# AIS-Bonn/stillleben

Measured on AMD Instinct MI355X. Metric: scenes/sec (settle + 640x480 6-ch GT render), 20-obj YCB-like, higher is better.
Workload: dtype f32; 1 GPU; C2: 20 of 21 procedural YCB-like objects (8k verts/16k tris, 1024^2 texture each) per scene; per step and GPU 32768 scenes are staged (random stack), settled (100 frames x 4 substeps), framed (camera, light, shadow matrix) and rendered at 640x480 (rgb, coord+depth, class, instance, normals; shadows on, SSAO on) -- all four stages inside the timed region; render_chunk=512, objects=20, settle_streams=1, render_streams=2, pair_contact_budget=0, parallelism=1 GPU

## Files before the change

### stillleben_amd/csrc/slhip_render.hip

```cpp
#include <vector>
#include <type_traits>
#include "slhip_common.h"
#include "slhip_cubemap.h"

#ifndef SLHIP_RENDER_WAVES
#define SLHIP_RENDER_WAVES 0
#endif
#ifndef SLHIP_SHADE_WAVES
#define SLHIP_SHADE_WAVES 0
#endif
#ifndef SLHIP_SSAO_WAVES
#define SLHIP_SSAO_WAVES 0
#endif
#if SLHIP_RENDER_WAVES > 0
#define SLHIP_LIGHT_KERNEL __attribute__((amdgpu_waves_per_eu(1, SLHIP_RENDER_WAVES)))
#else
#define SLHIP_LIGHT_KERNEL
#endif
#if SLHIP_SSAO_WAVES > 0
#define SLHIP_SSAO_KERNEL __attribute__((amdgpu_waves_per_eu(1, SLHIP_SSAO_WAVES)))
#else
#define SLHIP_SSAO_KERNEL
#endif
#if SLHIP_SHADE_WAVES > 0
// ... 996 lines not shown
                                                      const float4* __restrict__ clipbuf, unsigned n_clip_verts, int nl)
{
    const unsigned count = min(queue[0], capacity);
    const QItem* items = reinterpret_cast<const QItem*>(queue + 4);
    const unsigned lane = threadIdx.x & 63;
    const unsigned wave = (blockIdx.x * blockDim.x + threadIdx.x) >> 6;
    const unsigned n_waves = (gridDim.x * blockDim.x) >> 6;
    const unsigned per = (count + n_waves - 1) / n_waves;
    const unsigned i0 = wave * per, i1 = min(i0 + per, count);
    unsigned p_draw = 0xFFFFFFFFu, p_tri = 0u, p_scene = 0u;
    bool ok = false;
    Setup t;
    for (unsigned i = i0; i < i1; ++i) {
        const QItem it = items[i];
        if (it.draw == 0xFFFFFFFFu) continue;
        const unsigned scene = it.scene_aux & 0xFFFFFFu;
        const int light = (int)(it.scene_aux >> 24);
        if (it.draw != p_draw || it.tri_sub != p_tri || it.scene_aux != p_scene) {
            p_draw = it.draw; p_tri = it.tri_sub; p_scene = it.scene_aux;
            ok = false;
            const slhip_draw* dr = draws + it.draw;
            const unsigned* ip = pool.d_idx + dr->idx_base + 3 * (size_t)it.tri_sub;
            const float4* plane = clipbuf + (size_t)(1 + light) * n_clip_verts + dr->clip_base;
            const uint4* sp = reinterpret_cast<const uint4*>(plane);
            if (!setup_from_screen(sp[ip[0]], sp[ip[1]], sp[ip[2]], S, S, t)) continue;
            ok = true;
        }
        if (!ok) continue;
        const int px = (int)((it.tile & 0xFFFFu) << 3) + (int)(lane & 7);
        const int py = (int)((it.tile >> 16) << 3) + (int)(lane >> 3);
        if (px < t.xmin || px > t.xmax || py < t.ymin || py > t.ymax) continue;
        float l[3];
        if (!coverage(t, px, py, l)) continue;
        ShadowTarget tgt;
        tgt.win = nullptr; tgt.wx0 = 0; tgt.wy0 = 0;
        tgt.sm = shadow + ((size_t)scene * nl + light) * S * S;
        tgt.W = S;
        tgt.emit(t, px, py, l);
    }
}

__device__ __forceinline__ float frcp(float x) { return __builtin_amdgcn_rcpf(x); }
__device__ __forceinline__ void normalize3_fast(float* v)
{
    const float r = __builtin_amdgcn_rsqf(fmaf(v[2], v[2], fmaf(v[1], v[1], v[0] * v[0])));
    v[0] *= r; v[1] *= r; v[2] *= r;
}

__device__ __forceinline__ float distribution_ggx(const float* N, const float* Hv, float roughness)
{
    const float a = roughness * roughness;
    const float a2 = a * a;
    const float NdotH = fmaxf(dot3(N, Hv), 0.0f);
    const float NdotH2 = NdotH * NdotH;
    float denom = (NdotH2 * (a2 - 1.0f) + 1.0f);
    denom = kPi * denom * denom;
    return a2 * frcp(denom);
}

__device__ __forceinline__ float geometry_schlick_ggx(float NdotV, float roughness)
{
    const float r = roughness + 1.0f;
    const float k = (r * r) * 0.125f;
    return NdotV * frcp(NdotV * (1.0f - k) + k);
}

__device__ __forceinline__ float shadow_tap(const float* __restrict__ sm, int S, float u, float v, float ref)
{
    const float x = fmaf(u, (float)S, -0.5f), y = fmaf(v, (float)S, -0.5f);
    const float fx = floorf(x), fy = floorf(y);
    const float ax = x - fx, ay = y - fy;
    int x0 = (int)fx, y0 = (int)fy, x1 = x0 + 1, y1 = y0 + 1;
    x0 = min(max(x0, 0), S - 1); x1 = min(max(x1, 0), S - 1);
    y0 = min(max(y0, 0), S - 1); y1 = min(max(y1, 0), S - 1);
    const float r = clampf(ref, 0.0f, 1.0f);
    const float c00 = r <= sm[(size_t)y0 * S + x0] ? 1.0f : 0.0f;
    const float c10 = r <= sm[(size_t)y0 * S + x1] ? 1.0f : 0.0f;
    const float c01 = r <= sm[(size_t)y1 * S + x0] ? 1.0f : 0.0f;
    const float c11 = r <= sm[(size_t)y1 * S + x1] ? 1.0f : 0.0f;
    const float top = fmaf(ax, c10 - c00, c00), bot = fmaf(ax, c11 - c01, c01);
    return fmaf(ay, bot - top, top);
}

__device__ __forceinline__ float shadow_pcf16(const float* __restrict__ sm, int S, float px, float py, float ref,
                                              const unsigned* __restrict__ tile_bits)
{
    const float scale = 1.0f / (float)S;
    int ix[4], iy[4];
    float ax[4], ay[4];
    bool regular = true;
#pragma unroll
    for (int k = 0; k < 4; ++k) {
        const float o = (-1.5f + (float)k) * scale;
        const float x = fmaf(px + o, (float)S, -0.5f), y = fmaf(py + o, (float)S, -0.5f);
        const float fx = floorf(x), fy = floorf(y);
        ax[k] = x - fx; ay[k] = y - fy;
        ix[k] = (int)fx; iy[k] = (int)fy;
        if (k > 0 && (ix[k] != ix[0] + k || iy[k] != iy[0] + k)) regular = false;
    }
    float acc = 0.0f;
    if (regular) {
        const float r = clampf(ref, 0.0f, 1.0f);
        unsigned off_y[5];
        int cx[5];
#pragma unroll
        for (int k = 0; k < 5; ++k) {
            cx[k] = min(max(ix[0] + k, 0), S - 1);
            off_y[k] = (unsigned)min(max(iy[0] + k, 0), S - 1) * (unsigned)S;
        }
        if (tile_bits) {
            const int tn = shadow_tiles_x(S);
            const int ta = cx[0] / kShadowTile, tb = cx[4] / kShadowTile;
            const int ra = (int)(off_y[0] / (unsigned)S) / kShadowTile, rb = (int)(off_y[4] / (unsigned)S) / kShadowTile;
            const int t00 = ra * tn + ta, t01 = ra * tn + tb, t10 = rb * tn + ta, t11 = rb * tn + tb;
            const unsigned touched = ((tile_bits[t00 >> 5] >> (t00 & 31)) | (tile_bits[t01 >> 5] >> (t01 & 31)) |
                                      (tile_bits[t10 >> 5] >> (t10 & 31)) | (tile_bits[t11 >> 5] >> (t11 & 31))) & 1u;
            if (__ballot(touched == 0u) == __ballot(true)) return 1.0f;
        }
        bool lit[5][5];
        unsigned long long all_lit = ~0ull, any_lit = 0ull;
#pragma unroll
        for (int j = 0; j < 5; ++j)
#pragma unroll
            for (int i = 0; i < 5; ++i) {
                lit[j][i] = r <= sm[off_y[j] + (unsigned)cx[i]];
                const unsigned long long m = __ballot(lit[j][i]);
                all_lit &= m; any_lit |= m;
            }
        const unsigned long long here = __ballot(true);
        if (all_lit == here) return 1.0f;
        if (any_lit == 0ull) return 0.0f;
        float c[5][5];
#pragma unroll
        for (int j = 0; j < 5; ++j)
#pragma unroll
            for (int i = 0; i < 5; ++i) c[j][i] = lit[j][i] ? 1.0f : 0.0f;
#pragma unroll
        for (int yy = 0; yy < 4; ++yy)
#pragma unroll
            for (int xx = 0; xx < 4; ++xx) {
                const float top = fmaf(ax[xx], c[yy][xx + 1] - c[yy][xx], c[yy][xx]);
                const float bot = fmaf(ax[xx], c[yy + 1][xx + 1] - c[yy + 1][xx], c[yy + 1][xx]);
                acc += fmaf(ay[yy], bot - top, top);
            }
    } else {
        for (int yy = 0; yy < 4; ++yy)
            for (int xx = 0; xx < 4; ++xx) {
                const float ox = (-1.5f + (float)xx) * scale, oy = (-1.5f + (float)yy) * scale;
                acc += shadow_tap(sm, S, px + ox, py + oy, ref);
            }
    }
    return acc / 16.0f;
}

__device__ __forceinline__ float pow22(float x) { return __builtin_amdgcn_exp2f(2.2f * __builtin_amdgcn_logf(x)); }

__device__ __forceinline__ void shade_fragment(const slhip_scene* __restrict__ sc, const slhip_draw* __restrict__ dr,
                                               const float* base, const float* world, const float* nrm_in,
                                               bool front_facing, const float* __restrict__ shadow, int S, int shadow_lights,
                                               const unsigned* __restrict__ shadow_tiles, const slhip_light_map* __restrict__ lm, float roughness_in, float metallic_in,
                                               float occlusion, const float* emissive, float* color, float* normal_out)
{
    float normal[3] = {nrm_in[0], nrm_in[1], nrm_in[2]};
    if (!front_facing) { normal[0] = -normal[0]; normal[1] = -normal[1]; normal[2] = -normal[2]; }
    float V[3] = {sc->cam_position[0] - world[0], sc->cam_position[1] - world[1],
                  sc->cam_position[2] - world[2]};
    normalize3(V);
    const float NoV = clampf(dot3(normal, V), 1e-5f, 1.0f);
    const float roughness = fmaxf(roughness_in, 0.045f);
    const float metallic = metallic_in;

    color[0] = color[1] = color[2] = 0.0f;
    color[3] = base[3];

    float F0[3], kS[3];
    const float om = 1.0f - NoV, om2 = om * om;
    const float p5 = om2 * om2 * om;
#pragma unroll
    for (int c = 0; c < 3; ++c) {
        F0[c] = 0.04f * (1.0f - metallic) + base[c] * metallic;
        const float Fr = fmaxf(1.0f - roughness, F0[c]) - F0[c];
        kS[c] = F0[c] + Fr * p5;
    }
    const float base_pi[3] = {base[0] * (1.0f / kPi), base[1] * (1.0f / kPi), base[2] * (1.0f / kPi)};
    for (int i = 0; i < SLHIP_NUM_LIGHTS; ++i) {
        if (!light_active(sc, i)) continue;
        const float* lc = sc->light_color[i];
        const float* ld = sc->light_dir[i];
        float inverse_shadow = 1.0f;
        if (shadow && i < shadow_lights) {
            const float w4[4] = {world[0], world[1], world[2], 1.0f};
            float pc[4];
            mv4(sc->shadow_mat[i], w4, pc);
            const float rpw = 1.0f / pc[3];
            const float px = fmaf(pc[0] * rpw, 0.5f, 0.5f);
            const float py = fmaf(pc[1] * rpw, 0.5f, 0.5f);
            const float pz = fmaf(pc[2] * rpw, 0.5f, 0.5f);
            const float* sm = shadow + (size_t)i * S * S;
            inverse_shadow = shadow_pcf16(sm, S, px, py, (pz - 0.00003f), shadow_tiles ? shadow_tiles + (size_t)i * shadow_tile_words(S) : nullptr);
        }
        float L[3] = {-ld[0], -ld[1], -ld[2]};
        normalize3_fast(L);
        float Hv[3] = {V[0] + L[0], V[1] + L[1], V[2] + L[2]};
        normalize3_fast(Hv);
        const float NDF = distribution_ggx(normal, Hv, roughness);
        const float NdotVg = fmaxf(dot3(normal, V), 0.0f);
        const float NdotL = fmaxf(dot3(normal, L), 0.0f);
        const float G = geometry_schlick_ggx(NdotL, roughness) * geometry_schlick_ggx(NdotVg, roughness);
        const float denominator = fmaxf(4.0f * NoV * NdotL, 0.001f);
        const float rden = frcp(denominator);
#pragma unroll
        for (int c = 0; c < 3; ++c) {
            const float specular = (NDF * G * kS[c]) * rden;
            const float kD = (1.0f - kS[c]) * (1.0f - metallic);
            color[c] += inverse_shadow * (kD * base_pi[c] + specular) * lc[c] * NdotL;
        }
    }
#pragma unroll
    for (int c = 0; c < 3; ++c) color[c] += sc->ambient[c] * base[c];
    if (lm) {
        const float d2 = 2.0f * dot3(normal, V);
        const slcube::f3 refl = slcube::F3(d2 * normal[0] - V[0], d2 * normal[1] - V[1], d2 * normal[2] - V[2]);
        float fab[2];
        {
            const int n = (int)lm->lut_size;
            const float x = NoV * (float)n - 0.5f, y = roughness * (float)n - 0.5f;
            const float fx = floorf(x), fy = floorf(y);
            const float a = x - fx, b = y - fy;
            const int x0 = min(max((int)fx, 0), n - 1), x1 = min(max((int)fx + 1, 0), n - 1);
            const int y0 = min(max((int)fy, 0), n - 1), y1 = min(max((int)fy + 1, 0), n - 1);
            const float2* t = reinterpret_cast<const float2*>(lm->d_brdf_lut);
            const float2 c00 = t[y0 * n + x0], c10 = t[y0 * n + x1], c01 = t[y1 * n + x0], c11 = t[y1 * n + x1];
            const float tx = fmaf(a, c10.x - c00.x, c00.x), bx = fmaf(a, c11.x - c01.x, c01.x);
            const float ty = fmaf(a, c10.y - c00.y, c00.y), by = fmaf(a, c11.y - c01.y, c01.y);
            fab[0] = fmaf(b, bx - tx, tx); fab[1] = fmaf(b, by - ty, ty);
        }
        const float4 rad4 = slcube::sample_lod(lm->d_prefilter, lm->pre_size, lm->pre_levels, refl, roughness * 4.0f);
        const float4 irr4 = slcube::sample_lod(lm->d_irradiance, lm->irr_size, 1u, slcube::F3(normal[0], normal[1], normal[2]), 0.0f);
        const float rad[3] = {rad4.x, rad4.y, rad4.z}, irr[3] = {irr4.x, irr4.y, irr4.z};
        const float Ems = 1.0f - (fab[0] + fab[1]);
#pragma unroll
        for (int c = 0; c < 3; ++c) {
            const float c_diff = base[c] * (1.0f - 0.04f) * (1.0f - metallic);
            const float FssEss = kS[c] * fab[0] + fab[1];
            const float F_avg = F0[c] + (1.0f - F0[c]) / 21.0f;
            const float FmsEms = Ems * FssEss * F_avg / (1.0f - F_avg * Ems);
            const float k_D = c_diff * (1.0f - FssEss - FmsEms);
            color[c] += (FssEss * rad[c] + (FmsEms + k_D) * irr[c]) * occlusion;
        }
    }
#pragma unroll
    for (int c = 0; c < 3; ++c) color[c] += emissive[c];
    float nc[3];
#pragma unroll
    for (int r = 0; r < 3; ++r) {
        float a = fmaf(sc->world_to_cam[4 * r + 0], normal[0], 0.0f);
        a = fmaf(sc->world_to_cam[4 * r + 1], normal[1], a);
        a = fmaf(sc->world_to_cam[4 * r + 2], normal[2], a);
        nc[r] = a;
    }
    normalize3(nc);
    normal_out[0] = nc[0]; normal_out[1] = nc[1]; normal_out[2] = nc[2];
    normal_out[3] = dot3(normal, V);
}

__device__ __forceinline__ uchar4 tone_map_px(const float* c, float manual_exposure, float lum)
{
    const float X = 0.4124564f * c[0] + 0.3575761f * c[1] + 0.1804375f * c[2];
    float Y = 0.2126729f * c[0] + 0.7151522f * c[1] + 0.0721750f * c[2];
    const float Z = 0.0193339f * c[0] + 0.1191920f * c[1] + 0.9503041f * c[2];
    const float inv = frcp(X + Y + Z);
    const float xx = X * inv, yy = Y * inv;
    if (manual_exposure >= 0.0f) Y *= manual_exposure;
    else Y /= (9.6f * lum + 0.0001f);
    const float ryy = frcp(yy);
    const float x2 = Y * xx * ryy;
    const float y2 = Y;
    const float z2 = Y * (1.0f - xx - yy) * ryy;
    float o[3];
    o[0] = 3.2404542f * x2 + -1.5371385f * y2 + -0.4985314f * z2;
    o[1] = -0.9692660f * x2 + 1.8760108f * y2 + 0.0415560f * z2;
    o[2] = 0.0556434f * x2 + -0.2040259f * y2 + 1.0572252f * z2;
    unsigned char r[4];
#pragma unroll
    for (int k = 0; k < 3; ++k) {
        const float x = o[k];
        float v = (x * (2.51f * x + 0.03f)) * frcp(x * (2.43f * x + 0.59f) + 0.14f);
        v = fminf(fmaxf(v, 0.0f), 1.0f);
        if (!(v == v)) v = 0.0f;
        r[k] = (unsigned char)floorf(v * 255.0f + 0.5f);
    }
    const float a = fminf(fmaxf(c[3], 0.0f), 1.0f);
    r[3] = (unsigned char)floorf(a * 255.0f + 0.5f);
    return make_uchar4(r[0], r[1], r[2], r[3]);
}

__device__ __forceinline__ bool scene_block(unsigned blocks_per_scene, unsigned n_scenes, unsigned& scene, unsigned& blk)
{
    const unsigned x = blockIdx.x & 7u, j = blockIdx.x >> 3;
    scene = x + 8u * (j / blocks_per_scene);
    blk = j % blocks_per_scene;
    return scene < n_scenes;
}

struct PixelBary {
    float b[3], bx[3], by[3];
    bool front;
};
__device__ __forceinline__ bool resolve_pixel(const Setup& t, const float (&q0)[3], const float (&q1)[3], const float (&q2)[3],
                                              int px, int py, bool textured, PixelBary& r)
{
    float l[3];
    if (px < t.xmin || px > t.xmax || py < t.ymin || py > t.ymax) return false;
    if (!coverage(t, px, py, l)) return false;
    const float pw0 = l[0] * t.invw[0], pw1 = l[1] * t.invw[1], pw2 = l[2] * t.invw[2];
    const float sw = (pw0 + pw1) + pw2;
    const float bs[3] = {pw0 * (1.0f / sw), pw1 * (1.0f / sw), pw2 * (1.0f / sw)};
#pragma unroll
    for (int k = 0; k < 3; ++k) r.b[k] = fmaf(bs[2], q2[k], fmaf(bs[1], q1[k], bs[0] * q0[k]));
    r.front = t.flipped;
    if (textured) {
        bary_at(t, q0, q1, q2, px + 1, py, r.bx);
        bary_at(t, q0, q1, q2, px, py + 1, r.by);
    }
    return true;
}

struct ShadeParams {
    int W, H;
    unsigned n_scenes;
    unsigned flags;
    int S;
    int shadow_lights;
    int inline_tonemap;
    int want_lum;
    int tiled;
};

__global__ __launch_bounds__(256) SLHIP_SHADE_KERNEL void k_shade(slhip_mesh_pool pool, const slhip_scene* __restrict__ scenes,
                                               const slhip_draw* __restrict__ draws, ShadeParams prm,
                                               const unsigned long long* __restrict__ vis,
                                               slhip_render_out out, float* __restrict__ hdr,
                                               const float* __restrict__ shadow, float* __restrict__ lum_part,
                                               const float4* __restrict__ clipbuf, float* __restrict__ zplane,
                                               const float4* __restrict__ vattr, float2* __restrict__ ssao_tiles,
                                               const unsigned* __restrict__ shadow_tiles)
{
    const int W = prm.W, H = prm.H;
    const size_t P = (size_t)W * H;
    const unsigned blocks_per_scene = (unsigned)((P + 255) / 256);
    unsigned scene, blk;
    if (!scene_block(blocks_per_scene, prm.n_scenes, scene, blk)) return;
    unsigned pix;
    bool active;
    if (prm.tiled) {
        const unsigned per_row = (unsigned)W >> 5, l = threadIdx.x & 63u;
        const unsigned tx = (blk % per_row) * 32u + (threadIdx.x >> 6) * 8u + (l & 7u), ty = (blk / per_row) * 8u + (l >> 3);
        pix = ty * (unsigned)W + tx;
        active = true;
    } else {
        pix = blk * 256 + threadIdx.x;
        active = pix < P;
    }
    const slhip_scene* sc = scenes + scene;
    const size_t gp = (size_t)scene * P + pix;
    __shared__ unsigned s_prim_base[64];
    const unsigned n_scene_draws = sc->draw_end - sc->draw_begin;
    if (threadIdx.x < 64) s_prim_base[threadIdx.x] = threadIdx.x < n_scene_draws ? draws[sc->draw_begin + threadIdx.x].prim_base : 0xFFFFFFFFu;
    __syncthreads();

    const slhip_light_map* lm = (sc->light_map != 0u && pool.d_light_maps) ? pool.d_light_maps + (sc->light_map - 1u) : nullptr;
    float color[4] = {0.0f, 0.0f, 0.0f, 0.0f};
    float lum_color[4] = {0.0f, 0.0f, 0.0f, 0.0f};
    if (active) {
        const unsigned long long key = vis[gp];
        float coord[4] = {kInvalid, kInvalid, kInvalid, kInvalid};
        float camc[4] = {kInvalid, kInvalid, kInvalid, kInvalid};
        float nout[4] = {0.0f, 0.0f, 0.0f, 0.0f};
        float bary[4] = {0.0f, 0.0f, 0.0f, 0.0f};
        unsigned vidx[4] = {0u, 0u, 0u, 0u};
        unsigned cls = 0u, inst = 0u;
        bool plane_px = false;
        if (key != kVisEmpty) {
            const unsigned prim = (unsigned)(key & 0xFFFFFFFFull);
            unsigned d = sc->draw_begin;
            if (n_scene_draws <= 64) {
                unsigned lo = 0u;
#pragma unroll
                for (unsigned step = 32u; step > 0u; step >>= 1)
                    if (prim >= s_prim_base[lo + step]) lo += step;
                d = sc->draw_begin + lo;
            } else {
                for (unsigned i = sc->draw_begin + 1; i < sc->draw_end; ++i)
                    if (prim >= draws[i].prim_base) d = i;
            }
            const slhip_draw* dr = draws + d;
            const unsigned tri = prim - dr->prim_base;
            const unsigned* ip = pool.d_idx + dr->idx_base + 3 * (size_t)tri;
            const unsigned vi[3] = {ip[0], ip[1], ip[2]};
            VsOut vo[3];
            const int px = (int)(pix % (unsigned)W), py = (int)(pix / (unsigned)W);
            float b[3] = {0.0f, 0.0f, 0.0f}, bx[3] = {0.0f, 0.0f, 0.0f}, by[3] = {0.0f, 0.0f, 0.0f};
            bool found = false, front = false;
            uint4 sv[3] = {};
#pragma unroll
            for (int k = 0; k < 3; ++k) {
                const float4* va = vattr + 4 * (size_t)(dr->clip_base + vi[k]);
                const float4 a0 = va[0], a1 = va[1], a2 = va[2];
                sv[k] = reinterpret_cast<const uint4*>(va)[3];
                const float2 uv = reinterpret_cast<const float2*>(pool.d_uv)[dr->vtx_base + vi[k]];
                vo[k].objc[0] = a0.x; vo[k].objc[1] = a0.y; vo[k].objc[2] = a0.z; vo[k].objc[3] = a0.w;
                vo[k].world[0] = a1.x; vo[k].world[1] = a1.y; vo[k].world[2] = a1.z;
                vo[k].cam[0] = a1.w; vo[k].cam[1] = a2.w; vo[k].cam[2] = a0.w;
                vo[k].nrm[0] = a2.x; vo[k].nrm[1] = a2.y; vo[k].nrm[2] = a2.z;
                vo[k].uv[0] = uv.x; vo[k].uv[1] = uv.y;
            }
            const bool textured = (dr->flags & (SLHIP_DRAW_HAS_BASE_TEX | SLHIP_DRAW_HAS_NORMAL_TEX | SLHIP_DRAW_HAS_MR_TEX |
                                                SLHIP_DRAW_HAS_OCCLUSION_TEX | SLHIP_DRAW_HAS_EMISSIVE_TEX)) != 0u;
            PixelBary pb;
#pragma unroll
            for (int k = 0; k < 3; ++k) pb.b[k] = pb.bx[k] = pb.by[k] = 0.0f;
            pb.front = false;
            if (screen_all_inside(sv[0], sv[1], sv[2])) {
                const float e0[3] = {1.0f, 0.0f, 0.0f}, e1[3] = {0.0f, 1.0f, 0.0f}, e2[3] = {0.0f, 0.0f, 1.0f};
                Setup t;
                if (setup_from_screen(sv[0], sv[1], sv[2], W, H, t)) found = resolve_pixel(t, e0, e1, e2, px, py, textured, pb);
            } else {
                ClipVert cv[3];
#pragma unroll
                for (int k = 0; k < 3; ++k) {
                    const float4 c4 = clipbuf[dr->clip_base + vi[k]];
                    cv[k].clip[0] = c4.x; cv[k].clip[1] = c4.y; cv[k].clip[2] = c4.z; cv[k].clip[3] = c4.w;
                    cv[k].bary[0] = k == 0 ? 1.0f : 0.0f;
                    cv[k].bary[1] = k == 1 ? 1.0f : 0.0f;
                    cv[k].bary[2] = k == 2 ? 1.0f : 0.0f;
                }
                ClipVert poly[4];
                const int n = clip_near(cv, poly);
#pragma unroll
                for (int sub = 0; sub < 2; ++sub) {
                    if (sub >= n - 2 || found) break;
                    Setup t;
                    if (!setup_tri(poly[0].clip, poly[sub + 1].clip, poly[sub + 2].clip, W, H, t)) continue;
                    found = resolve_pixel(t, poly[0].bary, poly[sub + 1].bary, poly[sub + 2].bary, px, py, textured, pb);
                }
            }
            front = pb.front;
#pragma unroll
            for (int k = 0; k < 3; ++k) { b[k] = pb.b[k]; bx[k] = pb.bx[k]; by[k] = pb.by[k]; }
            if (found) {
                const float camz = interp(b, vo[0].objc[3], vo[1].objc[3], vo[2].objc[3]);
                float base[4] = {dr->base_color[0], dr->base_color[1], dr->base_color[2], dr->base_color[3]};
                const float u = interp(b, vo[0].uv[0], vo[1].uv[0], vo[2].uv[0]);
                const float v = interp(b, vo[0].uv[1], vo[1].uv[1], vo[2].uv[1]);
                const float dudx = interp(bx, vo[0].uv[0], vo[1].uv[0], vo[2].uv[0]) - u, dvdx = interp(bx, vo[0].uv[1], vo[1].uv[1], vo[2].uv[1]) - v;
                const float dudy = interp(by, vo[0].uv[0], vo[1].uv[0], vo[2].uv[0]) - u, dvdy = interp(by, vo[0].uv[1], vo[1].uv[1], vo[2].uv[1]) - v;
                if (dr->flags & SLHIP_DRAW_HAS_BASE_TEX) {
                    float tc[4];
                    tex_sample(pool.d_tex, dr->tex_offset, (int)dr->tex_w, (int)dr->tex_h, dr->tex_sampler[0], u, v, dudx, dvdx, dudy, dvdy, tc);
                    base[0] *= pow22(tc[0]);
                    base[1] *= pow22(tc[1]);
                    base[2] *= pow22(tc[2]);
                    base[3] *= tc[3];
                }
                float world[3], nrm[3];
#pragma unroll
                for (int k = 0; k < 3; ++k) {
                    world[k] = interp(b, vo[0].world[k], vo[1].world[k], vo[2].world[k]);
                    nrm[k] = interp(b, vo[0].nrm[k], vo[1].nrm[k], vo[2].nrm[k]);
                    coord[k] = interp(b, vo[0].objc[k], vo[1].objc[k], vo[2].objc[k]);
                    camc[k] = interp(b, vo[0].cam[k], vo[1].cam[k], vo[2].cam[k]);
                }
                coord[3] = camz;
                camc[3] = 1.0f;
                if (dr->flags & SLHIP_DRAW_HAS_STICKER) {
                    float sx[3], sy[3];
#pragma unroll
                    for (int k = 0; k < 3; ++k) {
                        const float4 p4 = reinterpret_cast<const float4*>(pool.d_pos)[dr->vtx_base + vi[k]];
                        const float pos[4] = {p4.x, p4.y, p4.z, 1.0f};
                        float obj4[4], sp[4];
                        mv4(dr->mesh_to_object, pos, obj4);
                        mv4(dr->sticker_projection, obj4, sp);
                        sx[k] = (sp[0] / sp[3] - dr->sticker_range[0]) / dr->sticker_range[2];
                        sy[k] = (sp[1] / sp[3] - dr->sticker_range[1]) / dr->sticker_range[3];
                    }
                    const float cx = interp(b, sx[0], sx[1], sx[2]), cy = interp(b, sy[0], sy[1], sy[2]);
                    if (cx >= 0.0f && cy >= 0.0f && cx < 1.0f && cy < 1.0f) {
                        float st[4];
                        tex_rect_bilinear(pool.d_tex + dr->sticker_tex_offset, (int)dr->sticker_tex_w, (int)dr->sticker_tex_h,
                                          cx * (float)dr->sticker_tex_w, cy * (float)dr->sticker_tex_h, st);
                        const float sc4[4] = {pow22(st[0]), pow22(st[1]), pow22(st[2]), st[3]};
#pragma unroll
                        for (int c = 0; c < 4; ++c) base[c] = base[c] * (1.0f - st[3]) + sc4[c] * st[3];
                    }
                }
                if (dr->flags & SLHIP_DRAW_HAS_NORMAL_TEX) {
                    float tw[3][3], bw[3][3];
#pragma unroll
                    for (int k = 0; k < 3; ++k) {
                        const float4 t4 = reinterpret_cast<const float4*>(pool.d_tan)[dr->vtx_base + vi[k]];
                        const float tv[3] = {t4.x, t4.y, t4.z};
                        mv3p(dr->normal_to_world, tv, tw[k]);
                        normalize3(tw[k]);
                        bw[k][0] = vo[k].nrm[1] * tw[k][2] - vo[k].nrm[2] * tw[k][1];
                        bw[k][1] = vo[k].nrm[2] * tw[k][0] - vo[k].nrm[0] * tw[k][2];
                        bw[k][2] = vo[k].nrm[0] * tw[k][1] - vo[k].nrm[1] * tw[k][0];
                        normalize3(bw[k]);
#pragma unroll
                        for (int c = 0; c < 3; ++c) bw[k][c] *= t4.w;
                    }
                    float tc[4];
                    tex_sample(pool.d_tex, dr->normal_tex_offset, (int)dr->normal_tex_w, (int)dr->normal_tex_h, dr->tex_sampler[1], u, v, dudx, dvdx, dudy, dvdy, tc);
                    const float nx = tc[0] * 2.0f - 1.0f, ny = tc[1] * 2.0f - 1.0f, nz = tc[2] * 2.0f - 1.0f;
                    float nn[3];
#pragma unroll
                    for (int c = 0; c < 3; ++c)
                        nn[c] = nx * interp(b, tw[0][c], tw[1][c], tw[2][c]) + ny * interp(b, bw[0][c], bw[1][c], bw[2][c]) + nz * nrm[c];
                    normalize3(nn);
                    nrm[0] = nn[0]; nrm[1] = nn[1]; nrm[2] = nn[2];
                }
                float roughness = dr->roughness, metallic = dr->metallic, occlusion = 1.0f;
                float emissive[3] = {dr->emissive[0], dr->emissive[1], dr->emissive[2]};
                if (dr->flags & SLHIP_DRAW_HAS_MR_TEX) {
                    float tc[4];
                    tex_sample(pool.d_tex, dr->mr_tex_offset, (int)dr->mr_tex_w, (int)dr->mr_tex_h, dr->tex_sampler[2], u, v, dudx, dvdx, dudy, dvdy, tc);
                    roughness *= tc[1];
                    metallic *= tc[2];
                }
                if (dr->flags & SLHIP_DRAW_HAS_OCCLUSION_TEX) {
                    float tc[4];
                    tex_sample(pool.d_tex, dr->occlusion_tex_offset, (int)dr->occlusion_tex_w, (int)dr->occlusion_tex_h, dr->tex_sampler[3], u, v, dudx, dvdx, dudy, dvdy, tc);
                    occlusion = tc[0];
                }
                if (dr->flags & SLHIP_DRAW_HAS_EMISSIVE_TEX) {
                    float tc[4];
                    tex_sample(pool.d_tex, dr->emissive_tex_offset, (int)dr->emissive_tex_w, (int)dr->emissive_tex_h, dr->tex_sampler[4], u, v, dudx, dvdx, dudy, dvdy, tc);
#pragma unroll
                    for (int c = 0; c < 3; ++c) emissive[c] *= pow22(tc[c]);
                }
                const float* sm = (prm.flags & SLHIP_RENDER_SHADOWS) && shadow
                                      ? shadow + (size_t)scene * prm.shadow_lights * prm.S * prm.S
                                      : nullptr;
                shade_fragment(sc, dr, base, world, nrm, front, sm, prm.S, prm.shadow_lights,
                               sm && shadow_tiles ? shadow_tiles + (size_t)scene * SLHIP_NUM_LIGHTS * shadow_tile_words(prm.S) : nullptr, lm, roughness, metallic, occlusion, emissive, color, nout);
                cls = dr->class_index & 0xFFFFu;
                inst = dr->instance_index & 0xFFFFu;
                plane_px = (dr->flags & (SLHIP_DRAW_NO_VERTEX_ID | SLHIP_DRAW_HAS_NORMAL_TEX)) == SLHIP_DRAW_NO_VERTEX_ID && inst == 0u;
                if (!(dr->flags & SLHIP_DRAW_NO_VERTEX_ID)) { vidx[0] = vi[0] + 1; vidx[1] = vi[1] + 1; vidx[2] = vi[2] + 1; }
                bary[0] = b[0]; bary[1] = b[1]; bary[2] = b[2];
            }
        }
#pragma unroll
        for (int c = 0; c < 4; ++c) lum_color[c] = color[c];
        if (key == kVisEmpty && sc->bg_tex[1] != 0u && sc->bg_tex[2] != 0u) {
            const int px = (int)(pix % (unsigned)W), py = (int)(pix / (unsigned)W);
            const int tw = (int)sc->bg_tex[1], th = (int)sc->bg_tex[2];
            const float tcx = ((float)px + 0.5f) / (float)W, tcy = 1.0f - ((float)py + 0.5f) / (float)H;
            float c[4];
            tex_rect_bilinear(pool.d_tex + sc->bg_tex[0], tw, th, (float)(int)(tcx * (float)tw), (float)(int)(tcy * (float)th), c);
            color[0] = c[0]; color[1] = c[1]; color[2] = c[2]; color[3] = 0.0f;
        } else if (key == kVisEmpty && lm) {
            const int px = (int)(pix % (unsigned)W), py = (int)(pix / (unsigned)W);
            const float xn = (2.0f * ((float)px + 0.5f)) / (float)W - 1.0f, yn = (2.0f * ((float)py + 0.5f)) / (float)H - 1.0f;
            const float dcx = (xn - sc->proj[2]) / sc->proj[0], dcy = (yn - sc->proj[6]) / sc->proj[5];
            const float* m = sc->world_to_cam;
            const slcube::f3 dw = slcube::F3(fmaf(m[8], 1.0f, fmaf(m[4], dcy, m[0] * dcx)), fmaf(m[9], 1.0f, fmaf(m[5], dcy, m[1] * dcx)),
                                            fmaf(m[10], 1.0f, fmaf(m[6], dcy, m[2] * dcx)));
            const float4 e = slcube::sample_lod(lm->d_env, lm->env_size, lm->env_levels, dw, 0.0f);
            color[0] = e.x; color[1] = e.y; color[2] = e.z; color[3] = 0.0f;
        }
        if (out.d_coord) reinterpret_cast<float4*>(out.d_coord)[gp] = make_float4(coord[0], coord[1], coord[2], coord[3]);
        if (out.d_class) out.d_class[gp] = (uint16_t)cls;
        if (out.d_instance) out.d_instance[gp] = (uint16_t)inst;
        if (out.d_normals) reinterpret_cast<float4*>(out.d_normals)[gp] = make_float4(nout[0], nout[1], nout[2], nout[3]);
        if (out.d_vertex_idx) reinterpret_cast<uint4*>(out.d_vertex_idx)[gp] = make_uint4(vidx[0], vidx[1], vidx[2], vidx[3]);
        if (out.d_bary) reinterpret_cast<float4*>(out.d_bary)[gp] = make_float4(bary[0], bary[1], bary[2], bary[3]);
        if (out.d_cam_coord) reinterpret_cast<float4*>(out.d_cam_coord)[gp] = make_float4(camc[0], camc[1], camc[2], camc[3]);
        if (zplane) {
            const int Wp = W + 2;
            float* zp = zplane + (size_t)scene * ((size_t)Wp * (H + 2));
            const int zi = (int)(pix % (unsigned)W), zj = (int)(pix / (unsigned)W);
            const int o = (zj + 1) * Wp + zi + 1;
            const float z = camc[2];
            const bool l = zi == 0, r = zi == W - 1, t = zj == 0, b = zj == H - 1;
            zp[o] = z;
            if (l) zp[o - 1] = z;
            if (r) zp[o + 1] = z;
            if (t) zp[o - Wp] = z;
            if (b) zp[o + Wp] = z;
            if (l && t) zp[o - Wp - 1] = z;
            if (r && t) zp[o - Wp + 1] = z;
            if (l && b) zp[o + Wp - 1] = z;
            if (r && b) zp[o + Wp + 1] = z;
        }
        if (ssao_tiles) {
            const bool geo = key != kVisEmpty;
            const unsigned long long other = __ballot(geo && !plane_px), any = __ballot(geo);
            float zm = geo ? camc[2] : 3.0e38f;
#pragma unroll
            for (int o = 32; o > 0; o >>= 1) zm = fminf(zm, __shfl_xor(zm, o, 64));
            if ((threadIdx.x & 63u) == 0u) {
                const unsigned tw = (unsigned)W >> 3;
                const unsigned tx = (pix % (unsigned)W) >> 3, ty = (pix / (unsigned)W) >> 3;
                ssao_tiles[(size_t)scene * (tw * ((unsigned)H >> 3)) + ty * tw + tx] =
                    make_float2(zm, __uint_as_float((other ? 1u : 0u) | (any ? 2u : 0u)));
            }
        }
        if (prm.inline_tonemap) {
            if (out.d_rgb) reinterpret_cast<uchar4*>(out.d_rgb)[gp] = tone_map_px(color, sc->manual_exposure, 0.0f);
        } else if (hdr) {
            reinterpret_cast<float4*>(hdr)[gp] = make_float4(color[0], color[1], color[2], color[3]);
        }
    }
    if (prm.want_lum) {
        __shared__ float red[4][256];
#pragma unroll
        for (int c = 0; c < 4; ++c) red[c][threadIdx.x] = lum_color[c];
        __syncthreads();
        for (int s = 128; s > 0; s >>= 1) {
            if (threadIdx.x < s) {
#pragma unroll
                for (int c = 0; c < 4; ++c) red[c][threadIdx.x] += red[c][threadIdx.x + s];
            }
            __syncthreads();
        }
        if (threadIdx.x < 4) lum_part[((size_t)scene * blocks_per_scene + blk) * 4 + threadIdx.x] = red[threadIdx.x][0];
    }
}

__constant__ float c_ssao_noise[48];
__constant__ float c_ssao_kernel[192];
// ... 155 lines not shown
    __shared__ float4 s_n[4][128];
    const unsigned bands = (unsigned)H >> 4;
    unsigned scene, rest;
    if (!scene_block(bands * 4u, n_scenes, scene, rest)) return;
    const unsigned band = rest >> 2, yc = rest & 3u, xc = threadIdx.x >> 6, lane = threadIdx.x & 63u;
    const size_t P = (size_t)W * H;
    const float* proj = scenes[scene].proj;
    const float* camS = zplane + (size_t)scene * ((size_t)(W + 2) * (H + 2));
    const int TW = W / kSsaoTile;
    const unsigned char* S = skip + (size_t)scene * ((size_t)TW * (H / kSsaoTile));
    const float4* N4 = reinterpret_cast<const float4*>(nrm) + (size_t)scene * P;
    const float4* C4 = reinterpret_cast<const float4*>(cam) + (size_t)scene * P;
    float* A = ao + (size_t)scene * P;
    unsigned* q = s_q[xc];
    float4* qn = s_n[xc];
    const unsigned per_row = (unsigned)W >> 2, total = 4u * per_row;
    unsigned count = 0;
    auto run = [&](unsigned n_run) {
        if (lane < n_run) {
            const unsigned pix = q[lane];
            const int i = (int)(pix % (unsigned)W), j = (int)(pix / (unsigned)W);
            A[pix] = ssao_pixel(proj, camS, W, H, i, j, qn[lane], C4[pix], kern);
        }
    };
    auto pixel_of = [&](unsigned ci) -> unsigned { return (band * 16u + yc + 4u * (ci / per_row)) * (unsigned)W + xc + 4u * (ci % per_row); };
    auto fetch = [&](unsigned ci, unsigned& pix, bool& sk, float4& n4) {
        pix = 0; sk = true; n4 = make_float4(0.0f, 0.0f, 0.0f, 0.0f);
        if (ci < total) {
            pix = pixel_of(ci);
            const unsigned y = pix / (unsigned)W, x = pix % (unsigned)W;
            sk = S[(y >> 3) * (unsigned)TW + (x >> 3)] != 0;
            if (!sk) n4 = N4[pix];
        }
    };
    unsigned pix_n; bool sk_n; float4 n4_n;
    fetch(lane, pix_n, sk_n, n4_n);
    for (unsigned c0 = 0; c0 < total; c0 += 64u) {
        const unsigned pix = pix_n;
        const bool sk = sk_n;
        const float4 n4 = n4_n;
        const bool valid = c0 + lane < total;
        fetch(c0 + 64u + lane, pix_n, sk_n, n4_n);
        const bool need = valid && !sk && !(n4.x == 0.0f && n4.y == 0.0f && n4.z == 0.0f);
        if (valid && !need) A[pix] = 1.0f;
        const unsigned long long m = __ballot(need);
        if (need) {
            const unsigned at = count + (unsigned)__popcll(m & ((1ull << lane) - 1ull));
            q[at] = pix; qn[at] = n4;
        }
        count += (unsigned)__popcll(m);
        __builtin_amdgcn_wave_barrier();
        if (count >= 64u) {
            run(64u);
            __builtin_amdgcn_wave_barrier();
            const unsigned left = count - 64u;
            unsigned mv = 0;
            float4 mn = make_float4(0.0f, 0.0f, 0.0f, 0.0f);
            if (lane < left) { mv = q[64u + lane]; mn = qn[64u + lane]; }
            __builtin_amdgcn_wave_barrier();
            if (lane < left) { q[lane] = mv; qn[lane] = mn; }
            count = left;
            __builtin_amdgcn_wave_barrier();
        }
    }
    if (count > 0u) run(count);
}

__global__ __launch_bounds__(256) SLHIP_LIGHT_KERNEL void k_ssao_apply(const slhip_scene* __restrict__ scenes, unsigned n_scenes, int W, int H,
                                                    const float* __restrict__ hdr_in, const float* __restrict__ ao,
                                                    const float* __restrict__ zplane, float* __restrict__ hdr_out,
                                                    const float* __restrict__ lum_scene, uint8_t* __restrict__ rgb,
                                                    const unsigned char* __restrict__ skip)
{
    const size_t P = (size_t)W * H;
    const unsigned blocks_per_scene = (unsigned)((P + 255) / 256);
    unsigned scene, blk;
    if (!scene_block(blocks_per_scene, n_scenes, scene, blk)) return;
    const unsigned pix = blk * 256 + threadIdx.x;
    if (pix >= P) return;
    const float* camS = zplane + (size_t)scene * ((size_t)(W + 2) * (H + 2));
    const float* aoS = ao + (size_t)scene * P;
    const size_t gp = (size_t)scene * P + pix;
    const int i = (int)(pix % (unsigned)W), j = (int)(pix / (unsigned)W);
    if (skip) {
        const int TW = W / kSsaoTile;
        const unsigned char* S = skip + (size_t)scene * ((size_t)TW * (H / kSsaoTile));
        const int xa = max(i - 2, 0) >> 3, xb = min(i + 1, W - 1) >> 3, ya = max(j - 2, 0) >> 3, yb = min(j + 1, H - 1) >> 3;
        const bool ones = (S[ya * TW + xa] & S[ya * TW + xb] & S[yb * TW + xa] & S[yb * TW + xb]) != 0;
        if (__all(ones)) {
            const float4 h = reinterpret_cast<const float4*>(hdr_in)[gp];
            const float c4[4] = {h.x, h.y, h.z, h.w};
            if (hdr_out) reinterpret_cast<float4*>(hdr_out)[gp] = h;
            if (rgb) {
                const float manual = scenes[scene].manual_exposure;
                const float lum = (manual >= 0.0f) ? 0.0f : lum_scene[(size_t)scene * blocks_per_scene * 4];
                reinterpret_cast<uchar4*>(rgb)[gp] = tone_map_px(c4, manual, lum);
            }
            return;
        }
    }
    const float sigma = 3.0f * 0.5f;
    const float falloff = 1.0f / (2.0f * sigma * sigma);
    unsigned rowo[5];
    int colx[5];
#pragma unroll
    for (int k = 0; k < 5; ++k) {
        colx[k] = min(max(i - 3 + k, 0), W - 1) + 1;
        rowo[k] = (unsigned)(min(max(j - 3 + k, 0), H - 1) + 1) * (unsigned)(W + 2);
    }
    float z[5][5];
#pragma unroll
    for (int r = 0; r < 5; ++r)
#pragma unroll
        for (int c = 0; c < 5; ++c) z[r][c] = camS[rowo[r] + (unsigned)colx[c]];
    auto corner = [&](int x, int y) {
        const float a = z[y + 2][x + 2], b = z[y + 2][x + 3], c = z[y + 3][x + 2], d = z[y + 3][x + 3];
        const float top = fmaf(0.5f, b - a, a), bot = fmaf(0.5f, d - c, c);
        return fmaf(0.5f, bot - top, top);
    };
    const float cd = corner(0, 0);
    float result = 0.0f, wt = 0.0f;
#pragma unroll
    for (int x = -2; x < 2; ++x)
#pragma unroll
        for (int y = -2; y < 2; ++y) {
            const int xi = min(max(i + x, 0), W - 1), yj = min(max(j + y, 0), H - 1);
            const float c = aoS[(unsigned)yj * (unsigned)W + (unsigned)xi];
            const float dz = corner(x, y);
            const float r = sqrtf((float)(x * x + y * y));
            const float dd = (dz - cd) * 300.0f;
            const float w = __builtin_amdgcn_exp2f(-r * r * falloff - dd * dd);
            wt += w;
            result += c * w;
        }
    const float a = result * frcp(wt);
    const float4 h = reinterpret_cast<const float4*>(hdr_in)[gp];
    const float c4[4] = {h.x * a, h.y * a, h.z * a, h.w};
    if (hdr_out) reinterpret_cast<float4*>(hdr_out)[gp] = make_float4(c4[0], c4[1], c4[2], c4[3]);
    if (rgb) {
        const float manual = scenes[scene].manual_exposure;
        const float lum = (manual >= 0.0f) ? 0.0f : lum_scene[(size_t)scene * blocks_per_scene * 4];
        reinterpret_cast<uchar4*>(rgb)[gp] = tone_map_px(c4, manual, lum);
    }
}

__global__ __launch_bounds__(256) void k_lum_reduce(const slhip_scene* __restrict__ scenes, unsigned blocks_per_scene, size_t P,
                                                    float* __restrict__ lum_part)
{
    const unsigned scene = blockIdx.x;
    if (scenes[scene].manual_exposure >= 0.0f) return;
    __shared__ float red[4][256];
    float acc[4] = {0.0f, 0.0f, 0.0f, 0.0f};
    float* part = lum_part + (size_t)scene * blocks_per_scene * 4;
    for (unsigned b = threadIdx.x; b < blocks_per_scene; b += 256)
#pragma unroll
        for (int c = 0; c < 4; ++c) acc[c] += part[4 * b + c];
#pragma unroll
    for (int c = 0; c < 4; ++c) red[c][threadIdx.x] = acc[c];
    __syncthreads();
    for (int s = 128; s > 0; s >>= 1) {
        if (threadIdx.x < s) {
#pragma unroll
            for (int c = 0; c < 4; ++c) red[c][threadIdx.x] += red[c][threadIdx.x + s];
        }
        __syncthreads();
    }
    if (threadIdx.x == 0) {
        const float inv = 1.0f / (float)P;
        const float a0 = red[0][0] * inv, a1 = red[1][0] * inv, a2 = red[2][0] * inv, a3 = red[3][0] * inv;
        part[0] = 0.1f * (0.2125f * (a0 / a3) + 0.7154f * (a1 / a3) + 0.0721f * (a2 / a3));
    }
}

__global__ __launch_bounds__(256) void k_tonemap(const slhip_scene* __restrict__ scenes, unsigned n_scenes, int W, int H,
                                                 const float* __restrict__ hdr, const float* __restrict__ lum_scene,
                                                 uint8_t* __restrict__ rgb)
{
    const size_t P = (size_t)W * H;
    const unsigned blocks_per_scene = (unsigned)((P + 255) / 256);
    unsigned scene, blk;
    if (!scene_block(blocks_per_scene, n_scenes, scene, blk)) return;
    const unsigned pix = blk * 256 + threadIdx.x;
    if (pix >= P) return;
    const float manual = scenes[scene].manual_exposure;
    const float lum = (manual >= 0.0f) ? 0.0f : lum_scene[(size_t)scene * blocks_per_scene * 4];
    const size_t gp = (size_t)scene * P + pix;
    const float4 h = reinterpret_cast<const float4*>(hdr)[gp];
    const float c[4] = {h.x, h.y, h.z, h.w};
    reinterpret_cast<uchar4*>(rgb)[gp] = tone_map_px(c, manual, lum);
}

__global__ __launch_bounds__(256) void k_clear_shadow(unsigned* __restrict__ shadow, size_t n4)
{
    uint4* p = reinterpret_cast<uint4*>(shadow);
    const uint4 v = make_uint4(0x3F800000u, 0x3F800000u, 0x3F800000u, 0x3F800000u);
    for (size_t i = (size_t)blockIdx.x * 256 + threadIdx.x; i < n4; i += (size_t)gridDim.x * 256) p[i] = v;
}

bool g_ssao_tables_uploaded[16] = {};

constexpr int kNumPhases = 8;
bool g_timing = false;
bool g_ev_created = false;
struct TimedCall { hipEvent_t ev[kNumPhases + 1]; bool recorded[kNumPhases + 1]; };
std::vector<TimedCall> g_timed;
TimedCall* g_cur = nullptr;
double g_acc_ms[kNumPhases] = {};

inline void mark(int i, hipStream_t stream)
{
    if (!g_timing || !g_cur) return;
    if (hipEventCreate(&g_cur->ev[i]) != hipSuccess) return;
    (void)hipEventRecord(g_cur->ev[i], stream);
    g_cur->recorded[i] = true;
}

}

extern "C" int slhip_timing_enable(int on)
// ... 255 lines not shown
```

Baseline: 9868 scenes/s.

## Stage draw tables and shadow tile bits in LDS for shading kernel

```diff
diff --git a/stillleben_amd/csrc/slhip_render.hip b/stillleben_amd/csrc/slhip_render.hip
--- a/stillleben_amd/csrc/slhip_render.hip
+++ b/stillleben_amd/csrc/slhip_render.hip
@@ -1102,8 +1102,16 @@
     return fmaf(ay, bot - top, top);
 }
 
+typedef const __attribute__((address_space(3))) unsigned* lds_bits_t;
+
+template <typename Bits>
+__device__ __forceinline__ unsigned shadow_tiles_touched(Bits bits, int t00, int t01, int t10, int t11)
+{
+    return ((bits[t00 >> 5] >> (t00 & 31)) | (bits[t01 >> 5] >> (t01 & 31)) | (bits[t10 >> 5] >> (t10 & 31)) | (bits[t11 >> 5] >> (t11 & 31))) & 1u;
+}
+
 __device__ __forceinline__ float shadow_pcf16(const float* __restrict__ sm, int S, float px, float py, float ref,
-                                              const unsigned* __restrict__ tile_bits)
+                                              const unsigned* __restrict__ tile_bits, lds_bits_t lds_bits)
 {
     const float scale = 1.0f / (float)S;
     int ix[4], iy[4];
@@ -1128,13 +1136,12 @@
             cx[k] = min(max(ix[0] + k, 0), S - 1);
             off_y[k] = (unsigned)min(max(iy[0] + k, 0), S - 1) * (unsigned)S;
         }
-        if (tile_bits) {
+        if (tile_bits || lds_bits) {
             const int tn = shadow_tiles_x(S);
             const int ta = cx[0] / kShadowTile, tb = cx[4] / kShadowTile;
             const int ra = (int)(off_y[0] / (unsigned)S) / kShadowTile, rb = (int)(off_y[4] / (unsigned)S) / kShadowTile;
             const int t00 = ra * tn + ta, t01 = ra * tn + tb, t10 = rb * tn + ta, t11 = rb * tn + tb;
-            const unsigned touched = ((tile_bits[t00 >> 5] >> (t00 & 31)) | (tile_bits[t01 >> 5] >> (t01 & 31)) |
-                                      (tile_bits[t10 >> 5] >> (t10 & 31)) | (tile_bits[t11 >> 5] >> (t11 & 31))) & 1u;
+            const unsigned touched = lds_bits ? shadow_tiles_touched(lds_bits, t00, t01, t10, t11) : shadow_tiles_touched(tile_bits, t00, t01, t10, t11);
             if (__ballot(touched == 0u) == __ballot(true)) return 1.0f;
         }
         bool lit[5][5];
@@ -1178,7 +1185,7 @@
 __device__ __forceinline__ void shade_fragment(const slhip_scene* __restrict__ sc, const slhip_draw* __restrict__ dr,
                                                const float* base, const float* world, const float* nrm_in,
                                                bool front_facing, const float* __restrict__ shadow, int S, int shadow_lights,
-                                               const unsigned* __restrict__ shadow_tiles, const slhip_light_map* __restrict__ lm, float roughness_in, float metallic_in,
+                                               const unsigned* __restrict__ shadow_tiles, lds_bits_t lds_tiles, const slhip_light_map* __restrict__ lm, float roughness_in, float metallic_in,
                                                float occlusion, const float* emissive, float* color, float* normal_out)
 {
     float normal[3] = {nrm_in[0], nrm_in[1], nrm_in[2]};
@@ -1217,7 +1224,8 @@
             const float py = fmaf(pc[1] * rpw, 0.5f, 0.5f);
             const float pz = fmaf(pc[2] * rpw, 0.5f, 0.5f);
             const float* sm = shadow + (size_t)i * S * S;
-            inverse_shadow = shadow_pcf16(sm, S, px, py, (pz - 0.00003f), shadow_tiles ? shadow_tiles + (size_t)i * shadow_tile_words(S) : nullptr);
+            inverse_shadow = shadow_pcf16(sm, S, px, py, (pz - 0.00003f), shadow_tiles ? shadow_tiles + (size_t)i * shadow_tile_words(S) : nullptr,
+                                          lds_tiles ? lds_tiles + i * shadow_tile_words(S) : nullptr);
         }
         float L[3] = {-ld[0], -ld[1], -ld[2]};
         normalize3_fast(L);
@@ -1384,16 +1392,38 @@
     }
     const slhip_scene* sc = scenes + scene;
     const size_t gp = (size_t)scene * P + pix;
-    __shared__ unsigned s_prim_base[64];
-    const unsigned n_scene_draws = sc->draw_end - sc->draw_begin;
-    if (threadIdx.x < 64) s_prim_base[threadIdx.x] = threadIdx.x < n_scene_draws ? draws[sc->draw_begin + threadIdx.x].prim_base : 0xFFFFFFFFu;
+    enum { kTabPrim, kTabIdx, kTabClip, kTabVtx, kTabFlags, kTabCols };
+    __shared__ unsigned s_draw[kTabCols][64];
+    __shared__ unsigned s_tile_bits[SLHIP_NUM_LIGHTS * kShadowMaxWords];
+    const unsigned draw_begin = sc->draw_begin, n_scene_draws = sc->draw_end - draw_begin;
+    const float* sm = (prm.flags & SLHIP_RENDER_SHADOWS) && shadow ? shadow + (size_t)scene * prm.shadow_lights * prm.S * prm.S : nullptr;
+    const unsigned tile_words = sm && shadow_tiles ? (unsigned)shadow_tile_words(prm.S) : 0u;
+    const bool tiles_in_lds = tile_words != 0u && tile_words <= (unsigned)kShadowMaxWords;
+    unsigned long long key = kVisEmpty;
+    if (active) key = vis[gp];
+    const bool tile_lane = tiles_in_lds && threadIdx.x < SLHIP_NUM_LIGHTS * tile_words;
+    unsigned bits = 0u;
+    if (tile_lane) bits = shadow_tiles[(size_t)scene * SLHIP_NUM_LIGHTS * tile_words + threadIdx.x];
+    {
+        const unsigned e = threadIdx.x & 63u, w = threadIdx.x >> 6;
+        unsigned v = w == kTabPrim ? 0xFFFFFFFFu : 0u, fl = 0u;
+        if (e < n_scene_draws) {
+            const slhip_draw* de = draws + draw_begin + e;
+            v = w == kTabPrim ? de->prim_base : w == kTabIdx ? de->idx_base : w == kTabClip ? de->clip_base : de->vtx_base;
+            fl = de->flags;
+        }
+        s_draw[w][e] = v;
+        if (w == 0u) s_draw[kTabFlags][e] = fl;
+        if (tile_lane) s_tile_bits[threadIdx.x] = bits;
+    }
     __syncthreads();
+    const unsigned* g_tiles = tile_words != 0u && !tiles_in_lds ? shadow_tiles + (size_t)scene * SLHIP_NUM_LIGHTS * tile_words : nullptr;
+    const lds_bits_t l_tiles = tiles_in_lds ? (lds_bits_t)s_tile_bits : nullptr;
 
     const slhip_light_map* lm = (sc->light_map != 0u && pool.d_light_maps) ? pool.d_light_maps + (sc->light_map - 1u) : nullptr;
     float color[4] = {0.0f, 0.0f, 0.0f, 0.0f};
     float lum_color[4] = {0.0f, 0.0f, 0.0f, 0.0f};
     if (active) {
-        const unsigned long long key = vis[gp];
         float coord[4] = {kInvalid, kInvalid, kInvalid, kInvalid};
         float camc[4] = {kInvalid, kInvalid, kInvalid, kInvalid};
         float nout[4] = {0.0f, 0.0f, 0.0f, 0.0f};
@@ -1403,21 +1433,31 @@
         bool plane_px = false;
         if (key != kVisEmpty) {
             const unsigned prim = (unsigned)(key & 0xFFFFFFFFull);
-            unsigned d = sc->draw_begin;
+            unsigned d = draw_begin;
+            unsigned d_prim_base, d_idx_base, d_clip_base, d_vtx_base, d_flags;
             if (n_scene_draws <= 64) {
                 unsigned lo = 0u;
 #pragma unroll
                 for (unsigned step = 32u; step > 0u; step >>= 1)
-                    if (prim >= s_prim_base[lo + step]) lo += step;
-                d = sc->draw_begin + lo;
+                    if (prim >= s_draw[kTabPrim][lo + step]) lo += step;
+                d = draw_begin + lo;
+                const lds_bits_t tab = (lds_bits_t)&s_draw[0][0] + lo;
+                d_prim_base = tab[kTabPrim * 64]; d_idx_base = tab[kTabIdx * 64]; d_clip_base = tab[kTabClip * 64];
+                d_vtx_base = tab[kTabVtx * 64]; d_flags = tab[kTabFlags * 64];
             } else {
-                for (unsigned i = sc->draw_begin + 1; i < sc->draw_end; ++i)
+                for (unsigned i = draw_begin + 1; i < sc->draw_end; ++i)
                     if (prim >= draws[i].prim_base) d = i;
+                d_prim_base = draws[d].prim_base; d_idx_base = draws[d].idx_base; d_clip_base = draws[d].clip_base;
+                d_vtx_base = draws[d].vtx_base; d_flags = draws[d].flags;
             }
             const slhip_draw* dr = draws + d;
-            const unsigned tri = prim - dr->prim_base;
-            const unsigned* ip = pool.d_idx + dr->idx_base + 3 * (size_t)tri;
+            const unsigned tri = prim - d_prim_base;
+            const unsigned* ip = pool.d_idx + d_idx_base + 3 * (size_t)tri;
             const unsigned vi[3] = {ip[0], ip[1], ip[2]};
+            const float d_base_color[4] = {dr->base_color[0], dr->base_color[1], dr->base_color[2], dr->base_color[3]};
+            const float d_roughness = dr->roughness, d_metallic = dr->metallic;
+            const float d_emissive[3] = {dr->emissive[0], dr->emissive[1], dr->emissive[2]};
+            const unsigned d_class = dr->class_index, d_instance = dr->instance_index;
             VsOut vo[3];
             const int px = (int)(pix % (unsigned)W), py = (int)(pix / (unsigned)W);
             float b[3] = {0.0f, 0.0f, 0.0f}, bx[3] = {0.0f, 0.0f, 0.0f}, by[3] = {0.0f, 0.0f, 0.0f};
@@ -1425,17 +1465,17 @@
             uint4 sv[3] = {};
 #pragma unroll
             for (int k = 0; k < 3; ++k) {
-                const float4* va = vattr + 4 * (size_t)(dr->clip_base + vi[k]);
+                const float4* va = vattr + 4 * (size_t)(d_clip_base + vi[k]);
                 const float4 a0 = va[0], a1 = va[1], a2 = va[2];
                 sv[k] = reinterpret_cast<const uint4*>(va)[3];
-                const float2 uv = reinterpret_cast<const float2*>(pool.d_uv)[dr->vtx_base + vi[k]];
+                const float2 uv = reinterpret_cast<const float2*>(pool.d_uv)[d_vtx_base + vi[k]];
                 vo[k].objc[0] = a0.x; vo[k].objc[1] = a0.y; vo[k].objc[2] = a0.z; vo[k].objc[3] = a0.w;
                 vo[k].world[0] = a1.x; vo[k].world[1] = a1.y; vo[k].world[2] = a1.z;
                 vo[k].cam[0] = a1.w; vo[k].cam[1] = a2.w; vo[k].cam[2] = a0.w;
                 vo[k].nrm[0] = a2.x; vo[k].nrm[1] = a2.y; vo[k].nrm[2] = a2.z;
                 vo[k].uv[0] = uv.x; vo[k].uv[1] = uv.y;
             }
-            const bool textured = (dr->flags & (SLHIP_DRAW_HAS_BASE_TEX | SLHIP_DRAW_HAS_NORMAL_TEX | SLHIP_DRAW_HAS_MR_TEX |
+            const bool textured = (d_flags & (SLHIP_DRAW_HAS_BASE_TEX | SLHIP_DRAW_HAS_NORMAL_TEX | SLHIP_DRAW_HAS_MR_TEX |
                                                 SLHIP_DRAW_HAS_OCCLUSION_TEX | SLHIP_DRAW_HAS_EMISSIVE_TEX)) != 0u;
             PixelBary pb;
 #pragma unroll
@@ -1449,7 +1489,7 @@
                 ClipVert cv[3];
 #pragma unroll
                 for (int k = 0; k < 3; ++k) {
-                    const float4 c4 = clipbuf[dr->clip_base + vi[k]];
+                    const float4 c4 = clipbuf[d_clip_base + vi[k]];
                     cv[k].clip[0] = c4.x; cv[k].clip[1] = c4.y; cv[k].clip[2] = c4.z; cv[k].clip[3] = c4.w;
                     cv[k].bary[0] = k == 0 ? 1.0f : 0.0f;
                     cv[k].bary[1] = k == 1 ? 1.0f : 0.0f;
@@ -1470,12 +1510,12 @@
             for (int k = 0; k < 3; ++k) { b[k] = pb.b[k]; bx[k] = pb.bx[k]; by[k] = pb.by[k]; }
             if (found) {
                 const float camz = interp(b, vo[0].objc[3], vo[1].objc[3], vo[2].objc[3]);
-                float base[4] = {dr->base_color[0], dr->base_color[1], dr->base_color[2], dr->base_color[3]};
+                float base[4] = {d_base_color[0], d_base_color[1], d_base_color[2], d_base_color[3]};
                 const float u = interp(b, vo[0].uv[0], vo[1].uv[0], vo[2].uv[0]);
                 const float v = interp(b, vo[0].uv[1], vo[1].uv[1], vo[2].uv[1]);
                 const float dudx = interp(bx, vo[0].uv[0], vo[1].uv[0], vo[2].uv[0]) - u, dvdx = interp(bx, vo[0].uv[1], vo[1].uv[1], vo[2].uv[1]) - v;
                 const float dudy = interp(by, vo[0].uv[0], vo[1].uv[0], vo[2].uv[0]) - u, dvdy = interp(by, vo[0].uv[1], vo[1].uv[1], vo[2].uv[1]) - v;
-                if (dr->flags & SLHIP_DRAW_HAS_BASE_TEX) {
+                if (d_flags & SLHIP_DRAW_HAS_BASE_TEX) {
                     float tc[4];
                     tex_sample(pool.d_tex, dr->tex_offset, (int)dr->tex_w, (int)dr->tex_h, dr->tex_sampler[0], u, v, dudx, dvdx, dudy, dvdy, tc);
                     base[0] *= pow22(tc[0]);
@@ -1493,11 +1533,11 @@
                 }
                 coord[3] = camz;
                 camc[3] = 1.0f;
-                if (dr->flags & SLHIP_DRAW_HAS_STICKER) {
+                if (d_flags & SLHIP_DRAW_HAS_STICKER) {
                     float sx[3], sy[3];
 #pragma unroll
                     for (int k = 0; k < 3; ++k) {
-                        const float4 p4 = reinterpret_cast<const float4*>(pool.d_pos)[dr->vtx_base + vi[k]];
+                        const float4 p4 = reinterpret_cast<const float4*>(pool.d_pos)[d_vtx_base + vi[k]];
                         const float pos[4] = {p4.x, p4.y, p4.z, 1.0f};
                         float obj4[4], sp[4];
                         mv4(dr->mesh_to_object, pos, obj4);
@@ -1515,11 +1555,11 @@
                         for (int c = 0; c < 4; ++c) base[c] = base[c] * (1.0f - st[3]) + sc4[c] * st[3];
                     }
                 }
-                if (dr->flags & SLHIP_DRAW_HAS_NORMAL_TEX) {
+                if (d_flags & SLHIP_DRAW_HAS_NORMAL_TEX) {
                     float tw[3][3], bw[3][3];
 #pragma unroll
                     for (int k = 0; k < 3; ++k) {
-                        const float4 t4 = reinterpret_cast<const float4*>(pool.d_tan)[dr->vtx_base + vi[k]];
+                        const float4 t4 = reinterpret_cast<const float4*>(pool.d_tan)[d_vtx_base + vi[k]];
                         const float tv[3] = {t4.x, t4.y, t4.z};
                         mv3p(dr->normal_to_world, tv, tw[k]);
                         normalize3(tw[k]);
@@ -1540,34 +1580,30 @@
                     normalize3(nn);
                     nrm[0] = nn[0]; nrm[1] = nn[1]; nrm[2] = nn[2];
                 }
-                float roughness = dr->roughness, metallic = dr->metallic, occlusion = 1.0f;
-                float emissive[3] = {dr->emissive[0], dr->emissive[1], dr->emissive[2]};
-                if (dr->flags & SLHIP_DRAW_HAS_MR_TEX) {
+                float roughness = d_roughness, metallic = d_metallic, occlusion = 1.0f;
+                float emissive[3] = {d_emissive[0], d_emissive[1], d_emissive[2]};
+                if (d_flags & SLHIP_DRAW_HAS_MR_TEX) {
                     float tc[4];
                     tex_sample(pool.d_tex, dr->mr_tex_offset, (int)dr->mr_tex_w, (int)dr->mr_tex_h, dr->tex_sampler[2], u, v, dudx, dvdx, dudy, dvdy, tc);
                     roughness *= tc[1];
                     metallic *= tc[2];
                 }
-                if (dr->flags & SLHIP_DRAW_HAS_OCCLUSION_TEX) {
+                if (d_flags & SLHIP_DRAW_HAS_OCCLUSION_TEX) {
                     float tc[4];
                     tex_sample(pool.d_tex, dr->occlusion_tex_offset, (int)dr->occlusion_tex_w, (int)dr->occlusion_tex_h, dr->tex_sampler[3], u, v, dudx, dvdx, dudy, dvdy, tc);
                     occlusion = tc[0];
                 }
-                if (dr->flags & SLHIP_DRAW_HAS_EMISSIVE_TEX) {
+                if (d_flags & SLHIP_DRAW_HAS_EMISSIVE_TEX) {
                     float tc[4];
                     tex_sample(pool.d_tex, dr->emissive_tex_offset, (int)dr->emissive_tex_w, (int)dr->emissive_tex_h, dr->tex_sampler[4], u, v, dudx, dvdx, dudy, dvdy, tc);
 #pragma unroll
                     for (int c = 0; c < 3; ++c) emissive[c] *= pow22(tc[c]);
                 }
-                const float* sm = (prm.flags & SLHIP_RENDER_SHADOWS) && shadow
-                                      ? shadow + (size_t)scene * prm.shadow_lights * prm.S * prm.S
-                                      : nullptr;
-                shade_fragment(sc, dr, base, world, nrm, front, sm, prm.S, prm.shadow_lights,
-                               sm && shadow_tiles ? shadow_tiles + (size_t)scene * SLHIP_NUM_LIGHTS * shadow_tile_words(prm.S) : nullptr, lm, roughness, metallic, occlusion, emissive, color, nout);
-                cls = dr->class_index & 0xFFFFu;
-                inst = dr->instance_index & 0xFFFFu;
-                plane_px = (dr->flags & (SLHIP_DRAW_NO_VERTEX_ID | SLHIP_DRAW_HAS_NORMAL_TEX)) == SLHIP_DRAW_NO_VERTEX_ID && inst == 0u;
-                if (!(dr->flags & SLHIP_DRAW_NO_VERTEX_ID)) { vidx[0] = vi[0] + 1; vidx[1] = vi[1] + 1; vidx[2] = vi[2] + 1; }
+                shade_fragment(sc, dr, base, world, nrm, front, sm, prm.S, prm.shadow_lights, g_tiles, l_tiles, lm, roughness, metallic, occlusion, emissive, color, nout);
+                cls = d_class & 0xFFFFu;
+                inst = d_instance & 0xFFFFu;
+                plane_px = (d_flags & (SLHIP_DRAW_NO_VERTEX_ID | SLHIP_DRAW_HAS_NORMAL_TEX)) == SLHIP_DRAW_NO_VERTEX_ID && inst == 0u;
+                if (!(d_flags & SLHIP_DRAW_NO_VERTEX_ID)) { vidx[0] = vi[0] + 1; vidx[1] = vi[1] + 1; vidx[2] = vi[2] + 1; }
                 bary[0] = b[0]; bary[1] = b[1]; bary[2] = b[2];
             }
         }
@@ -1889,13 +1925,13 @@
     const float* aoS = ao + (size_t)scene * P;
     const size_t gp = (size_t)scene * P + pix;
     const int i = (int)(pix % (unsigned)W), j = (int)(pix / (unsigned)W);
+    const float4 h = reinterpret_cast<const float4*>(hdr_in)[gp];
     if (skip) {
         const int TW = W / kSsaoTile;
         const unsigned char* S = skip + (size_t)scene * ((size_t)TW * (H / kSsaoTile));
         const int xa = max(i - 2, 0) >> 3, xb = min(i + 1, W - 1) >> 3, ya = max(j - 2, 0) >> 3, yb = min(j + 1, H - 1) >> 3;
         const bool ones = (S[ya * TW + xa] & S[ya * TW + xb] & S[yb * TW + xa] & S[yb * TW + xb]) != 0;
         if (__all(ones)) {
-            const float4 h = reinterpret_cast<const float4*>(hdr_in)[gp];
             const float c4[4] = {h.x, h.y, h.z, h.w};
             if (hdr_out) reinterpret_cast<float4*>(hdr_out)[gp] = h;
             if (rgb) {
@@ -1941,7 +1977,6 @@
             result += c * w;
         }
     const float a = result * frcp(wt);
-    const float4 h = reinterpret_cast<const float4*>(hdr_in)[gp];
     const float c4[4] = {h.x * a, h.y * a, h.z * a, h.w};
     if (hdr_out) reinterpret_cast<float4*>(hdr_out)[gp] = make_float4(c4[0], c4[1], c4[2], c4[3]);
     if (rgb) {
```

Result: no change. 9934 scenes/s (median of 6 runs) (+0.7%).
